# jurmy24/orb-slam3-rust

Measured on AMD Instinct MI355X. Metric: stereo frames/sec ORB extract+match @752x480, higher is better.
Workload: dtype u8; 1 GPU; Synthetic 752x480 stereo, 2000 ORB/frame, extract+match+triangulate (BASELINE configs[1]); n_features=2000, batch_pairs_per_gpu=512, distinct_batches=3, unique_pairs=1536, parallelism=frames sharded, 1 rank(s), no collective

## Files before the change

### orb-slam3-rust_amd/csrc/orb_kernels.hip

```cpp
#include <cfloat>
#include <cmath>

#include "orbx_internal.hpp"

namespace {

#include "orb_pattern_31.inc"

constexpr int EDGE = 31;

__constant__ __attribute__((aligned(16))) signed char c_pattern[256 * 4];

struct XcdMap { unsigned per_img, magic; };
__device__ __forceinline__ bool xcd_decode_at(XcdMap m, int n_img, unsigned L, int& img, int& b) {
  const unsigned x = L & 7u, slot = L >> 3;
  unsigned grp = __umulhi(slot, m.magic);
  unsigned r = slot - grp * m.per_img;
  if (r >= m.per_img) { ++grp; r -= m.per_img; }
  b = (int)r;
  img = (int)(grp * 8u + x);
  return img < n_img;
}
__device__ __forceinline__ bool xcd_decode(XcdMap m, int n_img, int& img, int& b) { return xcd_decode_at(m, n_img, blockIdx.x, img, b); }
static inline XcdMap xcd_map(int per_img) {
// ... 521 lines not shown
    acc_cnt = 0;
  };
  if (tid == 0) s_cnt = 0;
  for (int tile = tile0; tile < tile_end; ++tile) {
  const int img = cur.img, l = cur.l, x0 = cur.x0, y0 = cur.y0, w = cur.w, h = cur.h, aw = cur.aw, ah = cur.ah;
  if (tid == 0) s_npos = 0;
  const int qpr = (aw + 3) >> 2;
  const int ntask = qpr * ah;
  const unsigned inv = (unsigned)(65536.f / (float)qpr) + 1u;
#pragma unroll
  for (int k = 0; k < ST_PASS; ++k) {
    const int r = st_r0 + ST_RPP * k;
    if (st_r0 < ST_RPP && r < ah + 6) *reinterpret_cast<unsigned long long*>(&sp[r][8 * st_c]) = pf[k];
  }
#pragma unroll
  for (int i = tid; i < FS_W * FS_H / 16; i += FT_THREADS) reinterpret_cast<uint4*>(&ss[0][0])[i] = uint4{0u, 0u, 0u, 0u};
  __syncthreads();
  if (tile + 1 < tile_end) fetch(img0, tile + 1, nxt);
  const int t = g.fast_threshold;
  if (SWAR) {
    const int qpr16 = (aw + 15) >> 4;
    const int ntask16 = qpr16 * ah;
    const unsigned inv16 = (unsigned)(65536.f * __builtin_amdgcn_rcpf((float)qpr16)) + 1u;
    const unsigned T = (unsigned)t * 0x01010101u;
    const unsigned T1 = T + 0x01010101u;
    for (int task0 = 0; task0 < ntask16; task0 += FT_THREADS) {
      const int task = task0 + tid;
      unsigned m16 = 0;
      int j = 0, gq = 0;
      if (task < ntask16) {
        j = (int)(__umul24((unsigned)task, inv16) >> 16); gq = task - (int)__umul24((unsigned)j, (unsigned)qpr16);
        const uint2* crow = reinterpret_cast<const uint2*>(&sp[j + 3][16 * gq]);
        const uint2 c01 = crow[0], c23 = crow[1], c45 = crow[2];
        const unsigned* upr = reinterpret_cast<const unsigned*>(&sp[j][16 * gq + 4]);
        const unsigned* dnr = reinterpret_cast<const unsigned*>(&sp[j + 6][16 * gq + 4]);
        const unsigned up0 = upr[0], up1 = upr[1], up2 = upr[2], up3 = upr[3], dn0 = dnr[0], dn1 = dnr[1], dn2 = dnr[2], dn3 = dnr[3];
        const unsigned p0 = swar_compass_pass(c01.y, dn0, __builtin_amdgcn_alignbyte(c23.x, c01.y, 3), up0, __builtin_amdgcn_alignbyte(c01.y, c01.x, 1), T, T1);
        const unsigned p1 = swar_compass_pass(c23.x, dn1, __builtin_amdgcn_alignbyte(c23.y, c23.x, 3), up1, __builtin_amdgcn_alignbyte(c23.x, c01.y, 1), T, T1);
        const unsigned p2 = swar_compass_pass(c23.y, dn2, __builtin_amdgcn_alignbyte(c45.x, c23.y, 3), up2, __builtin_amdgcn_alignbyte(c23.y, c23.x, 1), T, T1);
        const unsigned p3 = swar_compass_pass(c45.x, dn3, __builtin_amdgcn_alignbyte(c45.y, c45.x, 3), up3, __builtin_amdgcn_alignbyte(c45.x, c23.y, 1), T, T1);
        m16 = ((((p0 >> 4) | p1) * 0x00204081u) >> 24) | (((((p2 >> 4) | p3) * 0x00204081u) >> 16) & 0xff00u);
      }
      const int cnt = __popc(m16);
      const int incl = wave_scan_incl(cnt);
      const int wtot = __builtin_amdgcn_readlane(incl, 63);
      if (wtot) {
        int base = 0;
        if (lane == 0) base = lds_add_rtn(&s_npos, wtot);
        int off = __builtin_amdgcn_readfirstlane(base) + incl - cnt;
        const unsigned short pbase = (unsigned short)(j * FS_W + 16 * gq);
        for (unsigned mm = m16; mm; mm &= mm - 1u) s_pos[off++] = (unsigned short)(pbase + (__ffs((int)mm) - 1));
      }
    }
  } else
  for (int task = tid; task < ntask; task += FT_THREADS) {
    const int j = (int)(__umul24((unsigned)task, inv) >> 16), tq = task - (int)__umul24((unsigned)j, (unsigned)qpr);
    const unsigned* rowc = reinterpret_cast<const unsigned*>(&sp[j + 3][0]) + tq;
    const unsigned c0 = rowc[0], c1 = rowc[1], c2 = rowc[2];
    const unsigned up = reinterpret_cast<const unsigned*>(&sp[j][0])[tq + 1];
    const unsigned dn = reinterpret_cast<const unsigned*>(&sp[j + 6][0])[tq + 1];
    const unsigned xm3 = __builtin_amdgcn_alignbyte(c1, c0, 1);
    const unsigned xp3 = __builtin_amdgcn_alignbyte(c2, c1, 3);
    const fast_s2 tt = {(short)t, (short)t};
    unsigned pass[2];
#pragma unroll
    for (int hf = 0; hf < 2; ++hf) {
      const unsigned sel = hf ? 0x0c030c02u : 0x0c010c00u;
      const fast_s2 v2 = __builtin_bit_cast(fast_s2, __builtin_amdgcn_perm(0u, c1, sel));
      const fast_s2 r0 = __builtin_bit_cast(fast_s2, __builtin_amdgcn_perm(0u, dn, sel));
      const fast_s2 r4 = __builtin_bit_cast(fast_s2, __builtin_amdgcn_perm(0u, xp3, sel));
      const fast_s2 r8 = __builtin_bit_cast(fast_s2, __builtin_amdgcn_perm(0u, up, sel));
      const fast_s2 r12 = __builtin_bit_cast(fast_s2, __builtin_amdgcn_perm(0u, xm3, sel));
      const fast_s2 B = __builtin_elementwise_min(__builtin_elementwise_max(r0, r8), __builtin_elementwise_max(r4, r12));
      const fast_s2 D = __builtin_elementwise_max(__builtin_elementwise_min(r0, r8), __builtin_elementwise_min(r4, r12));
      const fast_s2 eb = (v2 + tt) - B, ed = D - (v2 - tt);
      pass[hf] = (__builtin_bit_cast(unsigned, eb) | __builtin_bit_cast(unsigned, ed)) & 0x80008000u;
    }
    const bool pk0 = pass[0] & 0x8000u, pk1 = pass[0] & 0x80000000u, pk2 = pass[1] & 0x8000u, pk3 = pass[1] & 0x80000000u;
    const unsigned long long b0 = __ballot(pk0), b1 = __ballot(pk1), b2 = __ballot(pk2), b3 = __ballot(pk3);
    const int n0 = __popcll(b0), n1 = __popcll(b1), n2 = __popcll(b2), n3 = __popcll(b3);
    const int wtot = n0 + n1 + n2 + n3;
    if (wtot) {
      int base = 0;
      if (lane == 0) base = atomicAdd(&s_npos, wtot);
      base = __builtin_amdgcn_readfirstlane(base);
      const unsigned short p0 = (unsigned short)(j * FS_W + 4 * tq);
      if (pk0) s_pos[base + __builtin_amdgcn_mbcnt_hi((unsigned)(b0 >> 32), __builtin_amdgcn_mbcnt_lo((unsigned)b0, 0u))] = p0;
      base += n0;
      if (pk1) s_pos[base + __builtin_amdgcn_mbcnt_hi((unsigned)(b1 >> 32), __builtin_amdgcn_mbcnt_lo((unsigned)b1, 0u))] = p0 + 1;
      base += n1;
      if (pk2) s_pos[base + __builtin_amdgcn_mbcnt_hi((unsigned)(b2 >> 32), __builtin_amdgcn_mbcnt_lo((unsigned)b2, 0u))] = p0 + 2;
      base += n2;
      if (pk3) s_pos[base + __builtin_amdgcn_mbcnt_hi((unsigned)(b3 >> 32), __builtin_amdgcn_mbcnt_lo((unsigned)b3, 0u))] = p0 + 3;
    }
  }
  __syncthreads();
  const int npos = s_npos;
  if (acc_cnt > 0 && (acc_il != img * g.n_levels + l || acc_cnt + min(npos, FAST_LIST_CAP) > FAST_LIST_CAP)) append();
  for (int q = tid; q < npos; q += FT_THREADS) {
    const int p = s_pos[q], j = p >> 6, i = p & 63;
    const int cy = j + 3, cx = i + 4;
    const unsigned v = sp[cy][cx];
    unsigned r[16];
    r[0] = sp[cy + 3][cx];      r[1] = sp[cy + 3][cx + 1];  r[2] = sp[cy + 2][cx + 2];
    r[3] = sp[cy + 1][cx + 3];  r[4] = sp[cy][cx + 3];      r[5] = sp[cy - 1][cx + 3];
    r[6] = sp[cy - 2][cx + 2];  r[7] = sp[cy - 3][cx + 1];  r[8] = sp[cy - 3][cx];
    r[9] = sp[cy - 3][cx - 1];  r[10] = sp[cy - 2][cx - 2]; r[11] = sp[cy - 1][cx - 3];
    r[12] = sp[cy][cx - 3];     r[13] = sp[cy + 1][cx - 3]; r[14] = sp[cy + 2][cx - 2];
    r[15] = sp[cy + 3][cx - 1];
    const int hi = (int)v + t, lo = (int)v - t;
    const bool brighter = (int)min(max(r[0], r[8]), max(r[4], r[12])) > hi;
    const bool darker = (int)max(min(r[0], r[8]), min(r[4], r[12])) < lo;
    unsigned P[8];
#pragma unroll
    for (int k = 0; k < 8; ++k) P[k] = r[k] | (r[k + 8] << 16);
#ifdef ORBX_FAST_NO_LADDER
    int b = (int)((P[0] ^ P[1] ^ P[2] ^ P[3] ^ P[4] ^ P[5] ^ P[6] ^ P[7]) & 0xffu) + (brighter ? 1 : 0);
#else
    int b = fast_arc_score_h(v, P, brighter);
    if (brighter && darker) b = max(b, fast_arc_score_h(v, P, false));
#endif
    const int sc = b > t ? b - 1 : 0;
    ss[j][i] = (uint8_t)sc;
  }
  __syncthreads();
  for (int q = tid; q < npos; q += FT_THREADS) {
    const int p = s_pos[q];
    const int j = p >> 6, i = p & 63;
    const int x = x0 + i - 1, y = y0 + j - 1;
    const int sc = ss[j][i];
    const bool corner = sc > 0 && i >= 1 && i <= FT_W && j >= 1 && j <= FT_H && x < w - EDGE && y < h - EDGE;
    if (corner) {
      const int m = max(max(max((int)ss[j - 1][i - 1], (int)ss[j - 1][i]), max((int)ss[j - 1][i + 1], (int)ss[j][i - 1])),
                        max(max((int)ss[j][i + 1], (int)ss[j + 1][i - 1]), max((int)ss[j + 1][i], (int)ss[j + 1][i + 1])));
      if (sc > m) {
        const int pos = atomicAdd(&s_cnt, 1);
        if (pos < FAST_LIST_CAP) s_list[pos] = ((unsigned)sc << 24) | ((unsigned)y << 12) | (unsigned)x;
        else atomicOr(status, ORBX_ST_INTERNAL);
      }
    }
  }
  __syncthreads();
  acc_cnt = min(s_cnt, FAST_LIST_CAP);
  acc_il = img * g.n_levels + l;
  acc_off = g.lv[l].cand_off;
  acc_cap = g.lv[l].cand_cap;
  cur = nxt;
  }
  if (acc_cnt > 0) append();
}

__device__ __forceinline__ unsigned ld_u32(const uint8_t* p) {
  unsigned v;
  __builtin_memcpy(&v, p, 4);
  return v;
}

__device__ __forceinline__ float harris_response(const uint8_t* __restrict__ img, int pitch, int x0, int y0) {
  int a = 0, b = 0, c = 0;
  int rowm[9], row0[9], rowp[9];
  unsigned w[9][3];
#ifdef ORBX_HARRIS_UNALIGNED
  const uint8_t* p = img + (size_t)(y0 - 4) * pitch + (x0 - 4);
#pragma unroll
  for (int r = 0; r < 9; ++r) {
    const uint8_t* pr = p + (size_t)r * pitch;
    w[r][0] = ld_u32(pr); w[r][1] = ld_u32(pr + 4); w[r][2] = ld_u32(pr + 8);
  }
#else
  const unsigned sh = (unsigned)(x0 - 4) & 3u;
  const uint8_t* p = img + (unsigned)(__umul24((unsigned)(y0 - 4), (unsigned)pitch) + ((unsigned)(x0 - 4) & ~3u));
  struct alignas(4) Row12 { unsigned d[3]; };
  Row12 rw[9];
#pragma unroll
  for (int r = 0; r < 9; ++r) rw[r] = *reinterpret_cast<const Row12*>(p + (unsigned)r * (unsigned)pitch);
#pragma unroll
  for (int r = 0; r < 9; ++r) {
    w[r][0] = __builtin_amdgcn_alignbyte(rw[r].d[1], rw[r].d[0], sh);
    w[r][1] = __builtin_amdgcn_alignbyte(rw[r].d[2], rw[r].d[1], sh);
    w[r][2] = rw[r].d[2] >> (8u * sh);
  }
#endif
#define ORBX_ROW(dst, r)                                                                    \
  _Pragma("unroll") for (int k = 0; k < 4; ++k) {                                             \
    dst[k] = (int)((w[r][0] >> (8 * k)) & 0xffu);                                             \
    dst[4 + k] = (int)((w[r][1] >> (8 * k)) & 0xffu);                                         \
  }                                                                                           \
  dst[8] = (int)(w[r][2] & 0xffu);
  ORBX_ROW(rowm, 0)
  ORBX_ROW(row0, 1)
#pragma unroll
  for (int i = 0; i < 7; ++i) {
    ORBX_ROW(rowp, i + 2)
#pragma unroll
    for (int j = 0; j < 7; ++j) {
      const int Ix = (row0[j + 2] - row0[j]) * 2 + (rowm[j + 2] - rowm[j]) + (rowp[j + 2] - rowp[j]);
      const int Iy = (rowp[j + 1] - rowm[j + 1]) * 2 + (rowp[j] - rowm[j]) + (rowp[j + 2] - rowm[j + 2]);
      a += Ix * Ix; b += Iy * Iy; c += Ix * Iy;
    }
#pragma unroll
    for (int k = 0; k < 9; ++k) { rowm[k] = row0[k]; row0[k] = rowp[k]; }
  }
#undef ORBX_ROW
  const float scale = 1.f / (4 * 7 * 255.f);
  const float scale_sq_sq = scale * scale * scale * scale;
  const float fa = (float)a, fb = (float)b, fc = (float)c;
  const float t1 = __fmul_rn(fa, fb);
  const float t2 = __fmul_rn(fc, fc);
  const float sm = __fadd_rn(fa, fb);
  const float t3 = __fmul_rn(__fmul_rn(0.04f, sm), sm);
  float r = __fmul_rn(__fsub_rn(__fsub_rn(t1, t2), t3), scale_sq_sq);
  if (r == 0.f) r = 0.f;
  return r;
}

__device__ __forceinline__ unsigned orderable(float f) {
  const unsigned u = __float_as_uint(f);
  return (u & 0x80000000u) ? ~u : (u | 0x80000000u);
}
__device__ __forceinline__ float from_orderable(unsigned o) {
  const unsigned u = (o & 0x80000000u) ? (o & 0x7fffffffu) : ~o;
  return __uint_as_float(u);
}

struct HarrisPlan { int start[ORBX_MAX_LEVELS + 1]; };
__global__ __launch_bounds__(256) void harris_select_kernel(OrbSrc s, OrbGeom g, int n_img, XcdMap xm, const unsigned* __restrict__ cand,
                                                            const unsigned* __restrict__ cand_count,
                                                            const unsigned* __restrict__ hist,
                                                            unsigned long long* __restrict__ sel,
                                                            unsigned* __restrict__ sel_count, HarrisPlan hp) {
  __shared__ unsigned sh[256];
  __shared__ int s_thr;
  int img, bb;
  if (!xcd_decode(xm, n_img, img, bb)) return;
  int l = 0;
#pragma unroll
  for (int k = 1; k < ORBX_MAX_LEVELS; ++k) l += (bb >= hp.start[k]) ? 1 : 0;
  const int chunk = bb - hp.start[l], n_chunks = hp.start[l + 1] - hp.start[l];
  const int il = img * g.n_levels + l;
  const int tid = threadIdx.x;
  const unsigned count = min(cand_count[il], g.lv[l].cand_cap);
  const unsigned want = 2u * (unsigned)g.lv[l].quota;
  {
    const int lane = tid & 63, wave = tid >> 6;
    const unsigned hv = hist[(size_t)il * 256 + tid];
    const int incl = wave_scan_incl((int)hv);
    unsigned suf = (unsigned)(__builtin_amdgcn_readlane(incl, 63) - incl) + hv;
    if (lane == 0) sh[wave] = suf;
    if (tid == 0) s_thr = 0;
    __syncthreads();
    for (int w2 = wave + 1; w2 < 4; ++w2) suf += sh[w2];
    const unsigned long long m = __ballot(suf >= want);
    if (want == 0) { if (tid == 0) s_thr = 256; }
    else if (count > want && m && lane == 0) atomicMax(&s_thr, wave * 64 + 63 - __clzll((long long)m));
    __syncthreads();
  }
  const unsigned thr = (unsigned)s_thr;
  int pitch;
  const uint8_t* src = level_ptr(s, g, img, l, pitch);
  const unsigned* cl = cand + (size_t)img * g.cand_total + g.lv[l].cand_off;
  unsigned long long* out = sel + (size_t)img * g.cand_total + g.lv[l].cand_off;
  __shared__ unsigned s_pass[1024];
  __shared__ unsigned s_np;
  const int lane = tid & 63;
  const unsigned per = (count + (unsigned)n_chunks - 1u) / (unsigned)n_chunks;
  const unsigned lim = min(count, (chunk + 1) * per);
  for (unsigned base = chunk * per; base < lim; base += 1024u) {
    if (tid == 0) s_np = 0;
    __syncthreads();
#pragma unroll
    for (int k = 0; k < 4; ++k) {
      const unsigned i = base + k * 256 + tid;
      const unsigned c = i < lim ? cl[i] : 0u;
      const bool pass = i < lim && (c >> 24) >= thr;
      const unsigned long long m = __ballot(pass);
      if (m) {
        unsigned p0 = 0;
        if (lane == 0) p0 = (unsigned)lds_add_rtn(reinterpret_cast<int*>(&s_np), __popcll(m));
        p0 = __builtin_amdgcn_readfirstlane(p0);
        if (pass) s_pass[p0 + __builtin_amdgcn_mbcnt_hi((unsigned)(m >> 32), __builtin_amdgcn_mbcnt_lo((unsigned)m, 0u))] = c;
      }
    }
    __syncthreads();
    const unsigned np = s_np;
    unsigned mine = 0;
    for (unsigned q0 = (unsigned)(tid & ~63); q0 < np; q0 += 256) mine += min(64u, np - q0);
    unsigned pos0 = 0;
    if (lane == 0 && mine) pos0 = atomicAdd(&sel_count[il], mine);
    for (unsigned q0 = 0; q0 < np; q0 += 256) {
      const unsigned q = q0 + tid;
      if (q < np) {
        const unsigned c = s_pass[q];
        const int x = (int)(c & 0xfffu), y = (int)((c >> 12) & 0xfffu);
        const float r = harris_response(src, pitch, x, y);
        const unsigned long long key = ((unsigned long long)(~orderable(r)) << 32) | ((unsigned)y << 16) | (unsigned)x;
        out[__builtin_amdgcn_readfirstlane(pos0) + (q0 >> 8) * 64u + (unsigned)lane] = key;
      }
    }
    __syncthreads();
  }
}

constexpr int RK_NT = 256;
template <int E>
__device__ __forceinline__ void rank_pass(const unsigned long long* __restrict__ in, unsigned long long* __restrict__ out,
                                          unsigned M, unsigned g0, unsigned long long* chunk, int quota, unsigned* s_thr) {
  constexpr int CH = 2048;
  const int tid = threadIdx.x;
  unsigned long long my[E];
  unsigned rank[E];
#pragma unroll
  for (int e = 0; e < E; ++e) {
    const unsigned idx = g0 + e * RK_NT + tid;
    my[e] = idx < M ? in[idx] : ~0ull;
    rank[e] = 0;
  }
  for (unsigned c0 = 0; c0 < M; c0 += CH) {
    const unsigned n = min((unsigned)CH, M - c0);
    __syncthreads();
    for (unsigned i = tid; i < n; i += RK_NT) chunk[i] = in[c0 + i];
    __syncthreads();
    for (unsigned k = 0; k < n; ++k) {
      const unsigned long long v = chunk[k];
#pragma unroll
      for (int e = 0; e < E; ++e) rank[e] += (v < my[e]) ? 1u : 0u;
    }
  }
#pragma unroll
  for (int e = 0; e < E; ++e) {
    const unsigned idx = g0 + e * RK_NT + tid;
    if (idx < M) {
      out[rank[e]] = my[e];
      if ((int)rank[e] == quota - 1) *s_thr = (unsigned)(my[e] >> 32);
    }
  }
}

__device__ __forceinline__ void rank_prefix_1024(unsigned* skey, int tid) {
  constexpr int CE = 1024 / RK_NT;
  unsigned cv[CE], tot = 0;
#pragma unroll
  for (int q = 0; q < CE; ++q) { cv[q] = skey[CE * tid + q]; tot += cv[q]; }
  unsigned inc = tot;
#pragma unroll
  for (int off = 1; off < 64; off <<= 1) {
    const unsigned t = __shfl_up(inc, off);
    if ((tid & 63) >= off) inc += t;
  }
  if ((tid & 63) == 63) skey[1024 + (tid >> 6)] = inc;
  __syncthreads();
  unsigned run = inc - tot;
  for (int w = 0; w < (tid >> 6); ++w) run += skey[1024 + w];
#pragma unroll
  for (int q = 0; q < CE; ++q) { skey[CE * tid + q] = run; run += cv[q]; }
}

__global__ __launch_bounds__(RK_NT) void rank_select_kernel(OrbGeom g, int n_img, XcdMap xm, unsigned long long* __restrict__ sel,
                                                           const unsigned* __restrict__ sel_count,
                                                           unsigned long long* __restrict__ sel2,
                                                           unsigned* __restrict__ kept, uint2* __restrict__ tile_rng) {
  __shared__ unsigned long long chunk[2048];
  __shared__ unsigned skey[1024 + 16];
  __shared__ unsigned s_thr, s_keep;
  int img, l;
  if (!xcd_decode(xm, n_img, img, l)) return;
  const int il = img * g.n_levels + l;
  const int tid = threadIdx.x;
  const unsigned M = sel_count[il];
  const int quota = g.lv[l].quota;
  unsigned long long* in = sel + (size_t)img * g.cand_total + g.lv[l].cand_off;
  unsigned long long* out = sel2 + (size_t)img * g.cand_total + g.lv[l].cand_off;
  const bool tiled = g.dt_total > 0;
  const unsigned ntl = tiled ? (unsigned)(g.lv[l].dt_nx * g.lv[l].dt_ny) : 0u;
  uint2* rng = tile_rng + (size_t)img * (size_t)g.dt_total + g.lv[l].dt_start;
  const unsigned dt_nx = (unsigned)g.lv[l].dt_nx, dt_mx = g.lv[l].dt_mx, dt_my = g.lv[l].dt_my;
  auto tile_of = [&](unsigned xy) { return __umulhi((xy >> 16) - (unsigned)EDGE, dt_my) * dt_nx + __umulhi((xy & 0xffffu) - (unsigned)EDGE, dt_mx); };
  if (tid == 0) { s_thr = 0xffffffffu; s_keep = 0; }
  __syncthreads();
  if (M == 0 || quota == 0) {
    if (tid == 0) kept[il] = 0;
    for (unsigned t = tid; t < ntl; t += RK_NT) rng[t] = uint2{0u, 0u};
    return;
  }
  if (M <= 2048) {
    unsigned P = 128;
    while (P < M) P <<= 1;
    for (unsigned i = tid; i < P; i += RK_NT) chunk[i] = i < M ? in[i] : ~0ull;
    __syncthreads();
    unsigned pj = 128;
    for (unsigned k = 2; k <= P; k <<= 1) {
      for (unsigned j = k >> 1; j > 0; j >>= 1) {
        if (j >= 128 || pj >= 128) __syncthreads();
        else __builtin_amdgcn_fence(__ATOMIC_SEQ_CST, "workgroup");
        pj = j;
        for (unsigned c = tid; c < P / 2; c += RK_NT) {
          const unsigned i = ((c & ~(j - 1)) << 1) | (c & (j - 1));
          const unsigned ixj = i | j;
          const unsigned long long x = chunk[i], y = chunk[ixj];
          if ((x > y) == ((i & k) == 0)) { chunk[i] = y; chunk[ixj] = x; }
        }
      }
    }
    __syncthreads();
    for (unsigned i = tid; i < M; i += RK_NT) out[i] = chunk[i];
    if (M <= (unsigned)quota) {
      if (tid == 0) { kept[il] = M; s_keep = M; }
    } else {
      const unsigned thr = (unsigned)(chunk[quota - 1] >> 32);
      for (unsigned i = tid; i < M; i += RK_NT)
        if ((unsigned)(chunk[i] >> 32) <= thr && (i + 1 >= M || (unsigned)(chunk[i + 1] >> 32) > thr)) { kept[il] = i + 1; s_keep = i + 1; }
    }
    __syncthreads();
    const unsigned K = s_keep;
    int rsh = 4;
    while ((unsigned)(((g.lv[l].w + 127) >> 7) * ((g.lv[l].h >> rsh) + 1)) > 1024u) ++rsh;
    const unsigned nrb = (unsigned)(g.lv[l].h >> rsh) + 1u;
    for (int i = tid; i < 1024; i += RK_NT) skey[i] = 0u;
    __syncthreads();
    constexpr int KE = 2048 / RK_NT;
    unsigned mycell[KE], mypos[KE];
#pragma unroll
    for (int e = 0; e < KE; ++e) {
      const unsigned i = tid + (unsigned)RK_NT * e;
      if (i < K) {
        const unsigned xy = (unsigned)chunk[i];
        mycell[e] = tiled ? tile_of(xy) : ((xy & 0xffffu) >> 7) * nrb + ((xy >> 16) >> rsh);
        mypos[e] = atomicAdd(&skey[mycell[e]], 1u);
      }
    }
    __syncthreads();
    rank_prefix_1024(skey, tid);
    __syncthreads();
#pragma unroll
    for (int e = 0; e < KE; ++e) {
      const unsigned i = tid + (unsigned)RK_NT * e;
      if (i < K) in[skey[mycell[e]] + mypos[e]] = (chunk[i] & 0xffffffffull) | ((unsigned long long)i << 32);
    }
    for (unsigned t = tid; t < ntl; t += RK_NT) rng[t] = uint2{skey[t], t + 1 < ntl ? skey[t + 1] : K};
    return;
  }
  for (unsigned g0 = 0; g0 < M; g0 += 4 * RK_NT) rank_pass<4>(in, out, M, g0, chunk, quota, &s_thr);
  __syncthreads();
  unsigned K;
  if (M <= (unsigned)quota) {
    if (tid == 0) kept[il] = M;
    K = M;
  } else {
    const unsigned thr = s_thr;
    unsigned cnt = 0;
    for (unsigned i = tid; i < M; i += RK_NT) cnt += ((unsigned)(in[i] >> 32) <= thr) ? 1u : 0u;
    atomicAdd(&s_keep, cnt);
    __syncthreads();
    if (tid == 0) kept[il] = s_keep;
    K = min(s_keep, M);
  }
  __threadfence();
  __syncthreads();
  if (!tiled) {
    for (unsigned i = tid; i < K; i += RK_NT) in[i] = (out[i] & 0xffffffffull) | ((unsigned long long)i << 32);
    return;
  }
  unsigned* cursor = reinterpret_cast<unsigned*>(chunk);
  for (int i = tid; i < 1024; i += RK_NT) { skey[i] = 0u; cursor[i] = 0u; }
  __syncthreads();
  for (unsigned i = tid; i < K; i += RK_NT) atomicAdd(&skey[tile_of((unsigned)out[i])], 1u);
  __syncthreads();
  rank_prefix_1024(skey, tid);
  __syncthreads();
  for (unsigned i = tid; i < K; i += RK_NT) {
    const unsigned long long v = out[i];
    const unsigned c = tile_of((unsigned)v);
    in[skey[c] + atomicAdd(&cursor[c], 1u)] = (v & 0xffffffffull) | ((unsigned long long)i << 32);
  }
  for (unsigned t = tid; t < ntl; t += RK_NT) rng[t] = uint2{skey[t], t + 1 < ntl ? skey[t + 1] : K};
}

__device__ __forceinline__ float fast_atan2_deg(float y, float x) {
  const float p1 = 0.9997878412794807f * (float)(180 / 3.14159265358979323846);
  const float p3 = -0.3258083974640975f * (float)(180 / 3.14159265358979323846);
  const float p5 = 0.1555786518463281f * (float)(180 / 3.14159265358979323846);
  const float p7 = -0.04432655554792128f * (float)(180 / 3.14159265358979323846);
  const float ax = fabsf(x), ay = fabsf(y);
  float a, c, c2;
  if (ax >= ay) {
    c = __fdiv_rn(ay, __fadd_rn(ax, (float)DBL_EPSILON));
    c2 = __fmul_rn(c, c);
    a = __fmul_rn(__fadd_rn(__fmul_rn(__fadd_rn(__fmul_rn(__fadd_rn(__fmul_rn(p7, c2), p5), c2), p3), c2), p1), c);
  } else {
    c = __fdiv_rn(ax, __fadd_rn(ay, (float)DBL_EPSILON));
    c2 = __fmul_rn(c, c);
    a = __fsub_rn(90.f, __fmul_rn(__fadd_rn(__fmul_rn(__fadd_rn(__fmul_rn(__fadd_rn(__fmul_rn(p7, c2), p5), c2), p3), c2), p1), c));
  }
  if (x < 0) a = __fsub_rn(180.f, a);
  if (y < 0) a = __fsub_rn(360.f, a);
  return a;
}

__device__ __forceinline__ void sincos_deg(float angle_deg, float& c_out, float& s_out) {
  const float rad_f = __fmul_rn(angle_deg, (float)(3.14159265358979323846 / 180.f));
  const double t = (double)rad_f;
  const int k = (int)__dadd_rn(__dmul_rn(t, 0.63661977236758134308), 0.5);
  const double kd = (double)k;
  const double r = __dsub_rn(__dsub_rn(t, __dmul_rn(kd, 1.57079632673412561417e+00)), __dmul_rn(kd, 6.07710050650619224932e-11));
  const double z = __dmul_rn(r, r);
  double S = 1.0 / 355687428096000.0;
  S = __dsub_rn(__dmul_rn(S, z), 1.0 / 1307674368000.0);
  S = __dadd_rn(__dmul_rn(S, z), 1.0 / 6227020800.0);
  S = __dsub_rn(__dmul_rn(S, z), 1.0 / 39916800.0);
  S = __dadd_rn(__dmul_rn(S, z), 1.0 / 362880.0);
  S = __dsub_rn(__dmul_rn(S, z), 1.0 / 5040.0);
  S = __dadd_rn(__dmul_rn(S, z), 1.0 / 120.0);
  S = __dsub_rn(__dmul_rn(S, z), 1.0 / 6.0);
  const double sr = __dadd_rn(r, __dmul_rn(r, __dmul_rn(z, S)));
  double C = 1.0 / 20922789888000.0;
  C = __dsub_rn(__dmul_rn(C, z), 1.0 / 87178291200.0);
  C = __dadd_rn(__dmul_rn(C, z), 1.0 / 479001600.0);
  C = __dsub_rn(__dmul_rn(C, z), 1.0 / 3628800.0);
  C = __dadd_rn(__dmul_rn(C, z), 1.0 / 40320.0);
  C = __dsub_rn(__dmul_rn(C, z), 1.0 / 720.0);
  C = __dadd_rn(__dmul_rn(C, z), 1.0 / 24.0);
  C = __dsub_rn(__dmul_rn(C, z), 0.5);
  const double cr = __dadd_rn(1.0, __dmul_rn(z, C));
  double cs, sn;
  switch (k & 3) {
    case 0: cs = cr; sn = sr; break;
    case 1: cs = -sr; sn = cr; break;
    case 2: cs = -cr; sn = -sr; break;
    default: cs = sr; sn = -cr; break;
  }
  c_out = (float)cs;
  s_out = (float)sn;
}

__constant__ unsigned c_ic_ones[256];
__constant__ unsigned c_ic_col[256];

constexpr int DG_PER_WAVE = 4, DG_PER_BLOCK = 16;
typedef float desc_f2 __attribute__((ext_vector_type(2)));
__device__ __forceinline__ int row16_sum(int v) {
  v += __builtin_amdgcn_update_dpp(0, v, 0x128 , 0xf, 0xf, false);
  v += __builtin_amdgcn_update_dpp(0, v, 0x124 , 0xf, 0xf, false);
  v += __builtin_amdgcn_update_dpp(0, v, 0x122 , 0xf, 0xf, false);
  v += __builtin_amdgcn_update_dpp(0, v, 0x121 , 0xf, 0xf, false);
  return v;
}

constexpr int DF_WP = 48;
constexpr int DF_WIN_BYTES = 48 * DF_WP;
constexpr int DF_X0 = 23, DF_Y0 = 21;
typedef int df_i4 __attribute__((ext_vector_type(4)));
__constant__ __attribute__((aligned(16))) unsigned c_blur_band[6 * 64 * 4];
#ifndef ORBX_DF_ITERS
#define ORBX_DF_ITERS 2
#endif

__global__ __launch_bounds__(256) void describe_fused_kernel(OrbSrc s, OrbGeom g, int n_img, XcdMap xm, int blocks_per_img,
                                                             const unsigned long long* __restrict__ sel2,
                                                             const unsigned long long* __restrict__ spatial,
                                                             const unsigned* __restrict__ kept,
                                                             orbx_keypoint* __restrict__ kp_out, uint8_t* __restrict__ desc_out,
                                                             int* __restrict__ nkp, int cap_kp, float patch_size,
                                                             unsigned* __restrict__ status) {
  constexpr int kPatBytes = 1024;
  __shared__ __attribute__((aligned(16))) unsigned char s_win[DG_PER_BLOCK * DF_WIN_BYTES + kPatBytes + 2 * 1024];
  static_assert(sizeof(s_win) <= 40960, "four blocks per CU (160 KB of LDS)");
  int* s_pat = reinterpret_cast<int*>(s_win + DG_PER_BLOCK * DF_WIN_BYTES);
  unsigned* s_ones = reinterpret_cast<unsigned*>(s_win + DG_PER_BLOCK * DF_WIN_BYTES + kPatBytes);
  unsigned* s_col = s_ones + 256;
  int img, bx;
  if (!xcd_decode(xm, n_img, img, bx)) return;
  const int tid = threadIdx.x, lane = tid & 63, wave = tid >> 6;
  const int grp = lane >> 4, li = lane & 15;
  s_pat[tid] = reinterpret_cast<const int*>(c_pattern)[tid];
  s_ones[tid] = c_ic_ones[tid];
  s_col[tid] = c_ic_col[tid];
  __syncthreads();
  unsigned start[ORBX_MAX_LEVELS + 1];
  start[0] = 0;
#pragma unroll
  for (int l = 0; l < ORBX_MAX_LEVELS; ++l)
    start[l + 1] = start[l] + (l < g.n_levels ? kept[img * g.n_levels + l] : 0u);
  const unsigned total = start[ORBX_MAX_LEVELS];
  const unsigned limit = min(total, (unsigned)cap_kp);
  if (bx == 0 && tid == 0) {
    nkp[img] = (int)limit;
    if (total > (unsigned)cap_kp) atomicOr(status, ORBX_ST_KP_OVERFLOW);
  }
  unsigned char* wwin = s_win + wave * DG_PER_WAVE * DF_WIN_BYTES;
  unsigned char* mywin = wwin + grp * DF_WIN_BYTES;
  unsigned st_g[3], st_l[3];
#pragma unroll
  for (int ph = 0; ph < 3; ++ph) {
    const unsigned t0 = 16u * ph + (unsigned)li, r0 = (t0 * 171u) >> 10, c6 = t0 - 6u * r0;
    st_g[ph] = r0; st_l[ph] = r0 * DF_WP + 8u * c6;
  }
  const int l32 = lane & 31, hf = lane >> 5;
  for (unsigned base = (bx * 4 + wave) * DG_PER_WAVE; base < total; base += blocks_per_img * DG_PER_BLOCK) {
    const unsigned pos_raw = base + grp;
    const unsigned pos = pos_raw < total ? pos_raw : base;
    int l = 0;
    unsigned lbase = 0;
#pragma unroll
    for (int i = 1; i < ORBX_MAX_LEVELS; ++i) if (pos >= start[i]) { l = i; lbase = start[i]; }
    const size_t lofs = (size_t)img * g.cand_total + g.lv[l].cand_off;
    const unsigned long long ent = spatial[lofs + (pos - lbase)];
    const int kx = (int)(ent & 0xffffu), ky = (int)((ent >> 16) & 0xffffu);
    const unsigned j2 = (unsigned)(ent >> 32) & 0xffffu;
    const unsigned slot = lbase + j2;
    const bool active = pos_raw < total && slot < limit;
    const float resp = from_orderable(~(unsigned)(sel2[lofs + j2] >> 32));
    int pitch;
    const uint8_t* src = level_ptr(s, g, img, l, pitch);
    {
      const uint8_t* w0 = src + (unsigned)(__umul24((unsigned)(ky - DF_Y0), (unsigned)pitch) + (unsigned)(kx - DF_X0));
      const unsigned p8 = 8u * (unsigned)pitch;
      unsigned go[3];
#pragma unroll
      for (int ph = 0; ph < 3; ++ph) go[ph] = __umul24(st_g[ph], (unsigned)pitch) + (st_l[ph] - st_g[ph] * DF_WP);
      unsigned long long v[17];
#pragma unroll
      for (int it = 0; it < 17; ++it) {
        const int ph = it % 3, k = it / 3;
        if (it < 16 || li < 2) __builtin_memcpy(&v[it], w0 + (go[ph] + (unsigned)k * p8), 8);
      }
#pragma unroll
      for (int it = 0; it < 17; ++it) {
        const int ph = it % 3, k = it / 3;
        if (it < 16 || li < 2) *reinterpret_cast<unsigned long long*>(mywin + st_l[ph] + (unsigned)k * (8u * DF_WP)) = v[it] ^ 0x8080808080808080ull;
      }
    }
    __builtin_amdgcn_wave_barrier();
    __builtin_amdgcn_s_waitcnt(0);
    int sA = 0, sB = 0, sC = 0;
    {
      const unsigned char* c0 = mywin + ((li >> 2) + 6) * DF_WP + 8 + 8 * (li & 3);
#pragma unroll
      for (int it = 0; it < 8; ++it) {
        const int row = 4 * it + (li >> 2);
        const int r = min(row, 30);
        const unsigned long long px = *reinterpret_cast<const unsigned long long*>(c0 + (it * 4 - (row > 30 ? 1 : 0)) * DF_WP);
        const int t0 = row * 8 + 2 * (li & 3);
        const uint2 w1 = *reinterpret_cast<const uint2*>(&s_ones[t0]);
        const uint2 wc = *reinterpret_cast<const uint2*>(&s_col[t0]);
        const int sI = __builtin_amdgcn_sdot4((int)(px >> 32), (int)w1.y, __builtin_amdgcn_sdot4((int)px, (int)w1.x, 0, false), false);
        sA += __builtin_amdgcn_sdot4((int)(px >> 32), (int)wc.y, __builtin_amdgcn_sdot4((int)px, (int)wc.x, 0, false), false);
        sB += sI;
        sC += (r - 15) * sI;
      }
    }
    sA = row16_sum(sA); sB = row16_sum(sB); sC = row16_sum(sC);
    const int m10 = sA - 15 * sB, m01 = sC;
    const float angle = fast_atan2_deg((float)m01, (float)m10);
    float ca, sa;
    sincos_deg(angle, ca, sa);
    {
      const int m16 = lane & 15, q = lane >> 4;
      const df_i4* band = reinterpret_cast<const df_i4*>(c_blur_band) + lane;
#pragma unroll 1
      for (int kp = 0; kp < DG_PER_WAVE; ++kp) {
        unsigned char* win = wwin + kp * DF_WIN_BYTES;
        df_i4 a1[3];
#pragma unroll
        for (int mb = 0; mb < 3; ++mb) {
          a1[mb] = *reinterpret_cast<const df_i4*>(win + (16 * mb + m16) * DF_WP + 16 * q);
        }
        __builtin_amdgcn_s_waitcnt(0xc07f);
        __builtin_amdgcn_wave_barrier();
#pragma unroll
        for (int nb = 0; nb < 3; ++nb) {
          const df_i4 t1 = band[64 * nb];
          df_i4 hh[3];
#pragma unroll
          for (int mb = 0; mb < 3; ++mb) hh[mb] = __builtin_amdgcn_mfma_i32_16x16x64_i8(a1[mb], t1, (df_i4){0, 0, 0, 0}, 0, 0, 0);
          df_i4 bhi, blo;
#pragma unroll
          for (int mb = 0; mb < 3; ++mb) {
            const unsigned p01 = __builtin_amdgcn_perm((unsigned)hh[mb][1], (unsigned)hh[mb][0], 0x05010400u);
            const unsigned p23 = __builtin_amdgcn_perm((unsigned)hh[mb][3], (unsigned)hh[mb][2], 0x05010400u);
            blo[mb] = (int)(__builtin_amdgcn_perm(p23, p01, 0x05040100u) ^ 0x80808080u);
            bhi[mb] = (int)__builtin_amdgcn_perm(p23, p01, 0x07060302u);
          }
          blo[3] = 0; bhi[3] = 0;
#pragma unroll
          for (int mb2 = 0; mb2 < 3; ++mb2) {
            const df_i4 t2 = band[64 * (3 + mb2)];
            const df_i4 shi = __builtin_amdgcn_mfma_i32_16x16x64_i8(t2, bhi, (df_i4){0, 0, 0, 0}, 0, 0, 0);
            const df_i4 slo = __builtin_amdgcn_mfma_i32_16x16x64_i8(t2, blo, (df_i4){8454144, 8454144, 8454144, 8454144}, 0, 0, 0);
            const unsigned v0 = ((unsigned)shi[0] << 8) + (unsigned)slo[0], v1 = ((unsigned)shi[1] << 8) + (unsigned)slo[1];
            const unsigned v2 = ((unsigned)shi[2] << 8) + (unsigned)slo[2], v3 = ((unsigned)shi[3] << 8) + (unsigned)slo[3];
            const unsigned u01 = __builtin_amdgcn_perm(v1, v0, 0x00000602u), u23 = __builtin_amdgcn_perm(v3, v2, 0x00000602u);
            *reinterpret_cast<unsigned*>(win + (16 * nb + m16) * DF_WP + 16 * mb2 + 4 * q) = __builtin_amdgcn_perm(u23, u01, 0x05040100u);
          }
        }
      }
    }
    __builtin_amdgcn_wave_barrier();
    __builtin_amdgcn_s_waitcnt(0);
    typedef float desc_f4 __attribute__((ext_vector_type(4)));
    desc_f4 pat[8];
#pragma unroll
    for (int r = 0; r < 8; ++r) {
      const int pr = s_pat[8 * l32 + r];
      pat[r] = (desc_f4){(float)(signed char)(pr & 0xff), (float)(signed char)((pr >> 16) & 0xff), (float)(signed char)((pr >> 8) & 0xff), (float)(signed char)((pr >> 24) & 0xff)};
    }
    const desc_f2 magic2 = {12582912.f, 12582912.f};
    constexpr unsigned kBias = 0x400000u * DF_WP + 0x4B400000u - (18u * DF_WP + 18u);
    const unsigned slot_a = active ? slot : 0xffffffffu;
#pragma unroll
    for (int k2 = 0; k2 < 2; ++k2) {
      const int kp = 2 * k2 + hf;
      const int from = (16 * kp) << 2;
      const float cak = __int_as_float(__builtin_amdgcn_ds_bpermute(from, __float_as_int(ca)));
      const float sak = __int_as_float(__builtin_amdgcn_ds_bpermute(from, __float_as_int(sa)));
      const unsigned slotk = (unsigned)__builtin_amdgcn_ds_bpermute(from, (int)slot_a);
      const desc_f2 ca2 = {cak, cak}, sa2 = {sak, sak};
      const unsigned char* pbb = wwin + kp * DF_WIN_BYTES;
      const unsigned kbase = 0u - kBias;
      unsigned acc = 0;
#pragma unroll
      for (int r = 7; r >= 0; --r) {
        const desc_f2 X = {pat[r][0], pat[r][1]}, Y = {pat[r][2], pat[r][3]};
        const desc_f2 fx = X * ca2 - Y * sa2 + magic2;
        const desc_f2 fy = X * sa2 + Y * ca2 + magic2;
        unsigned a0, a1;
        asm("v_mad_u32_u24 %0, %1, %2, %3" : "=v"(a0) : "v"(__float_as_uint(fx[0])), "v"((unsigned)DF_WP), "v"(__float_as_uint(fy[0])));
        asm("v_mad_u32_u24 %0, %1, %2, %3" : "=v"(a1) : "v"(__float_as_uint(fx[1])), "v"((unsigned)DF_WP), "v"(__float_as_uint(fy[1])));
        const unsigned t0 = pbb[a0 + kbase];
        const unsigned t1 = pbb[a1 + kbase];
        acc = __builtin_amdgcn_alignbit(acc, t0 - t1, 31);
      }
      if (slotk != 0xffffffffu) desc_out[((size_t)img * cap_kp + slotk) * 32 + l32] = (uint8_t)acc;
    }
    if (active && li == 4) {
      const float sc = g.lv[l].scale;
      orbx_keypoint o;
      o.x = __fmul_rn((float)kx, sc);
      o.y = __fmul_rn((float)ky, sc);
      o.size = __fmul_rn(patch_size, sc);
      o.angle = angle;
      o.response = resp;
      o.octave = l;
      o.class_id = -1;
// ... 610 lines not shown
```

Baseline: 184,500 stereo frames/s.

## Radix-select quota threshold before bitonic sort to shrink sorted set and LDS

For levels with at most 2048 candidates, the kernel first finds the exact quota threshold with a four-pass 8-bit radix histogram select over register-held keys. It then compacts only the keys at or below that threshold into shared memory and bitonic-sorts that smaller set. This halves the chunk LDS array to 1024 entries by default, which is meant to cut sort work and raise occupancy. When ties push the kept count over the cap, it falls back to the rank pass, and the extra histogram passes and ballots add overhead on small inputs.

```diff
diff --git a/orb-slam3-rust_amd/csrc/orb_kernels.hip b/orb-slam3-rust_amd/csrc/orb_kernels.hip
--- a/orb-slam3-rust_amd/csrc/orb_kernels.hip
+++ b/orb-slam3-rust_amd/csrc/orb_kernels.hip
@@ -847,10 +847,15 @@
 }
 
 constexpr int RK_NT = 256;
+#ifndef ORBX_RK_CAP
+#define ORBX_RK_CAP 1024
+#endif
+constexpr int RK_CAP = ORBX_RK_CAP;
+static_assert(RK_CAP == 1024 || RK_CAP == 2048, "a power of two, at least the 1024 counters the tile sort keeps in the array, at most the 2048 keys held in registers");
 template <int E>
 __device__ __forceinline__ void rank_pass(const unsigned long long* __restrict__ in, unsigned long long* __restrict__ out,
                                           unsigned M, unsigned g0, unsigned long long* chunk, int quota, unsigned* s_thr) {
-  constexpr int CH = 2048;
+  constexpr int CH = RK_CAP;
   const int tid = threadIdx.x;
   unsigned long long my[E];
   unsigned rank[E];
@@ -904,8 +909,8 @@
                                                            const unsigned* __restrict__ sel_count,
                                                            unsigned long long* __restrict__ sel2,
                                                            unsigned* __restrict__ kept, uint2* __restrict__ tile_rng) {
-  __shared__ unsigned long long chunk[2048];
-  __shared__ unsigned skey[1024 + 16];
+  __shared__ unsigned long long chunk[RK_CAP];
+  __shared__ __attribute__((aligned(16))) unsigned skey[1024 + 16];
   __shared__ unsigned s_thr, s_keep;
   int img, l;
   if (!xcd_decode(xm, n_img, img, l)) return;
@@ -927,10 +932,78 @@
     for (unsigned t = tid; t < ntl; t += RK_NT) rng[t] = uint2{0u, 0u};
     return;
   }
+  constexpr int KL = 2048 / RK_NT;
+  unsigned long long my[KL];
+  unsigned Ksel = M;
   if (M <= 2048) {
+    const int lane = tid & 63;
+#pragma unroll
+    for (int e = 0; e < KL; ++e) {
+      const unsigned i = tid + (unsigned)RK_NT * e;
+      my[e] = i < M ? in[i] : ~0ull;
+    }
+    unsigned thr = 0xffffffffu;
+    if (M > (unsigned)quota) {
+      for (int i = tid; i < 1024; i += RK_NT) skey[i] = 0u;
+      __syncthreads();
+      unsigned prefix = 0, want = (unsigned)quota, hsel = 0;
+#pragma unroll
+      for (int p = 0; p < 4; ++p) {
+        const int shift = 24 - 8 * p;
+        unsigned* hist = skey + 256 * p;
+        const unsigned himask = p ? 0xffffffffu << (shift + 8) : 0u;
+#pragma unroll
+        for (int e = 0; e < KL; ++e) {
+          const unsigned hi = (unsigned)(my[e] >> 32);
+          const bool act = tid + (unsigned)RK_NT * e < M && ((hi ^ prefix) & himask) == 0u;
+          const unsigned d = (hi >> shift) & 255u;
+          const unsigned long long m = __ballot(act);
+          if (m) {
+            const int f = __ffsll((long long)m) - 1;
+            const unsigned d0 = (unsigned)__builtin_amdgcn_readlane((int)d, f);
+            if (__ballot(act && d != d0) == 0ull) { if (lane == f) atomicAdd(&hist[d0], (unsigned)__popcll(m)); }
+            else if (act) atomicAdd(&hist[d], 1u);
+          }
+        }
+        __syncthreads();
+        const uint4 h4 = reinterpret_cast<const uint4*>(hist)[lane];
+        const unsigned tot = h4.x + h4.y + h4.z + h4.w;
+        const unsigned incl = (unsigned)wave_scan_incl((int)tot);
+        const int L = __ffsll((long long)__ballot(incl >= want)) - 1;
+        unsigned w = want - (unsigned)__builtin_amdgcn_readlane((int)(incl - tot), L);
+        const unsigned b0 = (unsigned)__builtin_amdgcn_readlane((int)h4.x, L), b1 = (unsigned)__builtin_amdgcn_readlane((int)h4.y, L);
+        const unsigned b2 = (unsigned)__builtin_amdgcn_readlane((int)h4.z, L), b3 = (unsigned)__builtin_amdgcn_readlane((int)h4.w, L);
+        unsigned bin = 4u * (unsigned)L;
+        hsel = b0;
+        if (w > b0) { w -= b0; ++bin; hsel = b1; if (w > b1) { w -= b1; ++bin; hsel = b2; if (w > b2) { w -= b2; ++bin; hsel = b3; } } }
+        want = w;
+        prefix |= bin << shift;
+      }
+      thr = prefix;
+      Ksel = (unsigned)quota - want + hsel;
+    }
+    if (Ksel <= (unsigned)RK_CAP) {
+    const unsigned K = Ksel;
     unsigned P = 128;
-    while (P < M) P <<= 1;
-    for (unsigned i = tid; i < P; i += RK_NT) chunk[i] = i < M ? in[i] : ~0ull;
+    while (P < K) P <<= 1;
+    {
+      unsigned wtot = 0;
+#pragma unroll
+      for (int e = 0; e < KL; ++e)
+        wtot += (unsigned)__popcll(__ballot(tid + (unsigned)RK_NT * e < M && (unsigned)(my[e] >> 32) <= thr));
+      int base = 0;
+      if (lane == 0) base = lds_add_rtn(reinterpret_cast<int*>(&s_keep), (int)wtot);
+      base = __builtin_amdgcn_readfirstlane(base);
+#pragma unroll
+      for (int e = 0; e < KL; ++e) {
+        const bool keep = tid + (unsigned)RK_NT * e < M && (unsigned)(my[e] >> 32) <= thr;
+        const unsigned long long m = __ballot(keep);
+        const unsigned slot = (unsigned)base + __builtin_amdgcn_mbcnt_hi((unsigned)(m >> 32), __builtin_amdgcn_mbcnt_lo((unsigned)m, 0u));
+        if (keep && slot < (unsigned)RK_CAP) chunk[slot] = my[e];
+        base += __popcll(m);
+      }
+      for (unsigned i = K + tid; i < P; i += RK_NT) chunk[i] = ~0ull;
+    }
     __syncthreads();
     unsigned pj = 128;
     for (unsigned k = 2; k <= P; k <<= 1) {
@@ -947,22 +1020,14 @@
       }
     }
     __syncthreads();
-    for (unsigned i = tid; i < M; i += RK_NT) out[i] = chunk[i];
-    if (M <= (unsigned)quota) {
-      if (tid == 0) { kept[il] = M; s_keep = M; }
-    } else {
-      const unsigned thr = (unsigned)(chunk[quota - 1] >> 32);
-      for (unsigned i = tid; i < M; i += RK_NT)
-        if ((unsigned)(chunk[i] >> 32) <= thr && (i + 1 >= M || (unsigned)(chunk[i + 1] >> 32) > thr)) { kept[il] = i + 1; s_keep = i + 1; }
-    }
-    __syncthreads();
-    const unsigned K = s_keep;
+    for (unsigned i = tid; i < K; i += RK_NT) out[i] = chunk[i];
+    if (tid == 0) kept[il] = K;
     int rsh = 4;
     while ((unsigned)(((g.lv[l].w + 127) >> 7) * ((g.lv[l].h >> rsh) + 1)) > 1024u) ++rsh;
     const unsigned nrb = (unsigned)(g.lv[l].h >> rsh) + 1u;
     for (int i = tid; i < 1024; i += RK_NT) skey[i] = 0u;
     __syncthreads();
-    constexpr int KE = 2048 / RK_NT;
+    constexpr int KE = RK_CAP / RK_NT;
     unsigned mycell[KE], mypos[KE];
 #pragma unroll
     for (int e = 0; e < KE; ++e) {
@@ -983,6 +1048,8 @@
     }
     for (unsigned t = tid; t < ntl; t += RK_NT) rng[t] = uint2{skey[t], t + 1 < ntl ? skey[t + 1] : K};
     return;
+    }
+    __syncthreads();
   }
   for (unsigned g0 = 0; g0 < M; g0 += 4 * RK_NT) rank_pass<4>(in, out, M, g0, chunk, quota, &s_thr);
   __syncthreads();
```

New measurement: 186,500 stereo frames/s, median of 6. 1.1% higher.
